# KudanLimited/cuda-bundle-adjustment

Hardware: AMD Instinct MI355X
Metric: ba_edge_iterations_per_sec (higher is better)
Workload: dtype f64

## Files before the change

cuda-bundle-adjustment_amd/csrc/host/c_api.cpp:

```cpp
#include <cmath>
#include <cstring>
#include <deque>
#include <memory>
#include <unordered_map>

#include "../../../include/cugo_hip.h"
#include "../../include/cuda_graph_optimisation.h"
#include "../../include/icp_types.h"
#include "../../include/prior_types.h"
#include "../kernels/kernels.h"
#include "chol_solver.h"
#include "edge_layout.h"
#include "engine.h"
#include "hip_util.h"
#include "rccl_comm.h"
#include "schur_plan.h"

using namespace cugo_host;

namespace
{
template <typename F>
int guarded(F&& f)
{
// ... 311 lines not shown
{
    return guarded([&] { s->analyze(n, rowptr, colind); });
}
int cugo_chol_factor_solve(cugo_chol* s, const double* d_Hsc, double lambda, const double* d_bsc,
                           double* d_x, int32_t* d_fail)
{
    return guarded([&] {
        if (!s->analyzed || !s->ctx)
            throw std::runtime_error("cugo_chol_factor_solve needs an analysed solver with a device context");
        s->factor_solve(d_Hsc, lambda, d_bsc, d_x, d_fail);
    });
}
int cugo_chol_selected_inverse(cugo_chol* s, double* d_sigma)
{
    bool ok = true;
    const int rc = guarded([&] {
        if (!s || !s->ctx || !s->analyzed || !s->factored)
            throw std::runtime_error("cugo_chol_selected_inverse needs a factorisation (cugo_chol_factor_solve) since the "
                                     "last analyze()");
        if (s->own_subtrees())
            throw std::runtime_error("cugo_chol_selected_inverse: not available when the solver factors rank-owned "
                                     "subtrees");
        ok = s->selected_inverse(d_sigma);
    });
    if (rc != CUGO_OK)
        return rc;
    if (!ok)
    {
        set_last_error("cugo_chol_selected_inverse: the factorisation hit a zero pivot");
        return CUGO_ERR_NUMERIC;
    }
    return CUGO_OK;
}
#ifdef CUGO_DEBUG_HOOKS
int cugo_debug_pin_reference(void)
{
    return guarded([&] { cugo_debug_pin_reference_solver(); });
}
int cugo_debug_dump_call(int which, int call, const char* path)
{
    return guarded([&] {
        cugo_chol* s = cugo_debug_solver(which);
        if (!s)
            throw std::runtime_error("cugo_debug_dump_call: no solver has run with CUGO_DEBUG_KEEP");
        s->dump_slot(call, path);
    });
}
int cugo_debug_plan_array(int which, const char* name, const int32_t** out)
{
    cugo_chol* s = cugo_debug_solver(which);
    if (!s)
        return -1;
    return cugo_chol_plan_array(s, name, out);
}
int cugo_debug_dump(const char* dir, int* n_calls)
{
    return guarded([&] {
        const int n = cugo_debug_dump_last_solver(dir);
        if (n_calls)
            *n_calls = n;
    });
}
#endif
int cugo_chol_stats(const cugo_chol* s, double* nnzL, double* flops, int* n_super, int* n_stages,
                    double* front_bytes)
{
// ... 694 lines not shown
```

cuda-bundle-adjustment_amd/csrc/host/chol_solver.cpp:

```cpp
#include "chol_solver.h"

#include <cstdio>
#include <cstdlib>
#include <cstring>
#include <string>

using namespace cugo_host;

void cugo_chol::pack()
{
    const CholPlan& P = plan;
    pack32.clear(), pack64.clear();
    auto put32 = [this](const std::vector<int32_t>& v) {
        const size_t o = pack32.size();
        pack32.insert(pack32.end(), v.begin(), v.end());
        pack32.resize((pack32.size() + 3) & ~size_t(3));
        return o;
    };
    auto put64 = [this](const std::vector<int64_t>& v) {
        const size_t o = pack64.size();
        pack64.insert(pack64.end(), v.begin(), v.end());
        pack64.resize((pack64.size() + 1) & ~size_t(1));
        return o;
    };
    const size_t o_ncb = put32(P.ncb), o_nb = put32(P.nb), o_col0 = put32(P.col0);
    const size_t o_alias = put32(P.alias_of), o_bwnp = put32(P.bw_np), o_lanp = put32(P.la_np);
    const size_t o_rows_ptr = put32(P.rows_ptr), o_rows = put32(P.rows);
    const size_t o_child_ptr = put32(P.child_ptr), o_child = put32(P.child);
    const size_t o_rel_ptr = put32(P.rel_ptr), o_rel = put32(P.rel);
    const size_t o_task_ptr = put32(P.task_ptr), o_task_fronts = put32(P.task_fronts);
    const size_t o_blk_front = put32(P.blk_front), o_blk_row = put32(P.blk_row), o_blk_col = put32(P.blk_col);
    const size_t o_perm = put32(P.perm), o_col_front = put32(P.col_front), o_wl = put32(P.wl);
    const size_t ntask = P.task_ptr.empty() ? 0 : P.task_ptr.size() - 1;
    constexpr int R = cugo_k::EA1_REC;
// ... 85 lines not shown
    }
    for (size_t k = 0; k < P.bc_seg.size() / 3; k++)
        std::memcpy(bc_seg.data() + 4 * k, P.bc_seg.data() + 3 * k, 3 * sizeof(int32_t));
    const size_t o_bc_rec = put32(bc_rec), o_bc_seg = put32(bc_seg);
    const size_t o_asm_map = put32(P.asm_map);
    const size_t o_trans = pack32.size();
    pack32.resize(o_trans + (P.blk_trans.size() + 3) / 4 + 4, 0);
    if (!P.blk_trans.empty())
        std::memcpy(pack32.data() + o_trans, P.blk_trans.data(), P.blk_trans.size());
    const size_t o_asm_off = put64(P.asm_off);
    const size_t o_off = put64(P.off), o_woff = put64(P.woff), o_l21off = put64(P.l21off), o_ldf = put64(P.ldf);
    po = {o_ncb, o_nb, o_col0, o_alias, o_bwnp, o_lanp, o_rows_ptr, o_rows, o_child_ptr, o_child, o_rel_ptr, o_rel,
          o_task_ptr, o_task_fronts, o_blk_front, o_blk_row, o_blk_col, o_perm, o_col_front, o_wl, o_ea1, o_tmeta,
          o_fat, o_asm_map, o_trans, o_asm_off, o_off, o_woff, o_l21off, o_ldf, o_bc_rec, o_bc_seg};
}

void cugo_chol::upload(hipStream_t s)
{
    const CholPlan& P = plan;
    const size_t o_ncb = po[0], o_nb = po[1], o_col0 = po[2], o_alias = po[3], o_bwnp = po[4], o_lanp = po[5];
    const size_t o_rows_ptr = po[6], o_rows = po[7], o_child_ptr = po[8], o_child = po[9], o_rel_ptr = po[10];
    const size_t o_rel = po[11], o_task_ptr = po[12], o_task_fronts = po[13], o_blk_front = po[14], o_blk_row = po[15];
    const size_t o_blk_col = po[16], o_perm = po[17], o_col_front = po[18], o_wl = po[19], o_ea1 = po[20];
    const size_t o_tmeta = po[21], o_fat = po[22], o_asm_map = po[23], o_trans = po[24], o_asm_off = po[25];
    const size_t o_off = po[26], o_woff = po[27], o_l21off = po[28], o_ldf = po[29];
    const size_t o_bc_rec = po[30], o_bc_seg = po[31];
    d_pack32.upload(pack32, s), d_pack64.upload(pack64, s);
    d_fronts.resize((size_t)P.front_doubles + 16);
    d_fronts.zero(s);
    d_xnew.resize((size_t)6 * P.n + 16);
    d_junk.resize(64 * 1024);
    d_winv.resize((size_t)P.winv_doubles + 16);
    d_l21.resize((size_t)P.l21_doubles + 16);
    bw_chain = opt.bw_chain && !opt.lookahead && !P.has_subtree_stage && !P.bc_front.empty();
    if (bw_chain)
    {
        d_bc_state.resize((size_t)cugo_k::BC_DONE + P.n_super);
        d_bc_state.zero(s);
        h_bc_error.resize(1);
        h_bc_error[0] = 0;
        bc_base = 0, bc_epoch = 0;
    }
    CUGO_HIP(hipStreamSynchronize(s));

    cugo_k::CholPlanDev& D = dev;
    D.n_fronts = P.n_super;
    const int32_t* b32 = d_pack32.data();
    const int64_t* b64 = d_pack64.data();
    D.ncb = b32 + o_ncb, D.nb = b32 + o_nb, D.off = b64 + o_off, D.col0 = b32 + o_col0;
    D.rows_ptr = b32 + o_rows_ptr, D.rows = b32 + o_rows;
    D.child_ptr = b32 + o_child_ptr, D.child = b32 + o_child;
    D.rel_ptr = b32 + o_rel_ptr, D.rel = b32 + o_rel;
    D.n_stages = P.n_stages;
    D.task_ptr = b32 + o_task_ptr, D.task_fronts = b32 + o_task_fronts, D.tmeta = b32 + o_tmeta;
    D.n_hsc_blocks = (int)P.blk_front.size();
    D.blk_front = b32 + o_blk_front, D.blk_row = b32 + o_blk_row;
    D.blk_col = b32 + o_blk_col, D.blk_trans = reinterpret_cast<const uint8_t*>(b32 + o_trans);
    D.n = P.n, D.perm = b32 + o_perm, D.col_front = b32 + o_col_front;
    D.junk = d_junk.data();
    D.woff = b64 + o_woff, D.winv = d_winv.data(), D.nc_max = P.nc_max;
    D.ea_lds = opt.ea_lds, D.panel16 = opt.panel16, D.ea_direct = opt.ea_direct;
#ifdef CUGO_DEBUG_HOOKS
    {
        const char* ka = std::getenv("CUGO_KERNEL_ACQUIRE");
        D.kernel_acquire = ka ? std::atoi(ka) & 7 : 0;
        const char* ed = std::getenv("CUGO_DEBUG_DELAY");
        D.dbg_delay = ed ? std::atoi(ed) : 0;
        const char* ez = std::getenv("CUGO_DEBUG_ZERO_LDS");
        D.zero_lds = ez ? std::atoi(ez) : 0, D.lds_doubles = 0;
        D.dbg_skip_wg = -1;
    }
#endif
    D.l21off = b64 + o_l21off, D.l21 = d_l21.data();
    D.ldf = b64 + o_ldf, D.alias_of = b32 + o_alias, D.bw_np = b32 + o_bwnp, D.la_np = b32 + o_lanp;
// ... 136 lines not shown
                    if (plan.woff[k] <= e && plan.woff[k] >= plan.woff[f])
                        f = k;
                stale_line = c.d_winv.data() + e, stale_stage = stage_of[f], stale_kind = 0;
            }
            else if (kind == 1 && e + 16 <= 6LL * plan.n)
                stale_line = c.d_xnew.data() + e, stale_stage = stage_of[plan.col_front[e / 6]], stale_kind = 1;
            if (stale_line)
            {
                c.dbg_scratch.resize(16);
                CUGO_HIP(hipMemcpyAsync(c.dbg_scratch.data(), stale_line, 16 * sizeof(double), hipMemcpyDeviceToDevice, s));
            }
        }
    }
    ~cugo_chol_hooks()
    {
        if (skip_on)
            cugo_k::chol_dbg_skip_end();
    }
    void hash(int slot, const double* ptr, size_t n)
    {
        if (c.dbg_hash && slot < 64)
            cugo_k::launch_hash_words(s, ptr, n, c.dbg_hash + slot);
    }
    void after_level(int st)
    {
        if (hash_levels && st < 24)
        {
            hash(16 + st, c.d_winv.data(), (size_t)c.plan.winv_doubles);
            hash(40 + st, c.d_fronts.data(), (size_t)c.plan.front_doubles);
        }
        if (gap)
            cugo_k::launch_nop(s);
    }
    double* stale_for_potrf(int st) const { return stale_kind == 0 && stale_stage == st ? stale_line : nullptr; }
    void after_two_phase(int st)
    {
        if (stale_kind == 0 && stale_stage == st)
            cugo_k::launch_swap16(s, stale_line, c.dbg_scratch.data());
    }
    void after_backward(int st)
    {
        if (stale_kind == 1 && (st == stale_stage || st == stale_stage - 1))
            cugo_k::launch_swap16(s, stale_line, c.dbg_scratch.data());
    }
    void keep_arrays(double* d_x)
    {
        if (!keep_on || c.dbg_calls > 16)
            return;
        const cugo_host::CholPlan& plan = c.plan;
        const size_t nf = (size_t)plan.front_doubles, nw = (size_t)plan.winv_doubles, nl = (size_t)plan.l21_doubles,
                     nx = (size_t)6 * plan.n;
        while (c.keep.size() < (size_t)c.dbg_calls)
            c.keep.emplace_back(new cugo_host::DevBuf<double>());
        auto& k = *c.keep[c.dbg_calls - 1];
        k.resize(nf + nw + nl + 2 * nx + 8);
        double* dst = k.data();
        const std::pair<const double*, size_t> parts[] = {{c.d_fronts.data(), nf}, {c.d_winv.data(), nw}, {c.d_l21.data(), nl},
                                                          {c.d_xnew.data(), nx}, {d_x, nx}};
        for (const auto& pr : parts)
        {
            if (pr.second)
                CUGO_HIP(hipMemcpyAsync(dst, pr.first, pr.second * sizeof(double), hipMemcpyDeviceToDevice, s));
            dst += pr.second;
        }
        g_last_kept = &c;
    }
};
#define CUGO_HOOK(expr) expr
#else
cugo_chol::~cugo_chol() {}
#define CUGO_HOOK(expr) ((void)0)
#endif

void cugo_chol::factor_solve(const double* d_Hsc, double lambda, const double* d_bsc, double* d_x,
                             int32_t* d_fail)
{
    hipStream_t s = ctx->stream;
    check_chain_error();
    factored = true, last_fail = d_fail;
#ifdef CUGO_DEBUG_HOOKS
    cugo_chol_hooks hooks(*this);
#endif
#ifdef CUGO_STAMPS
    static const bool dbg = std::getenv("CUGO_DEBUG_STAMPS") != nullptr;
    static long long* d_stamps = nullptr;
    if (dbg && !d_stamps)
    {
        CUGO_HIP(hipMalloc(reinterpret_cast<void**>(&d_stamps), 64 * sizeof(long long)));
        CUGO_HIP(hipMemset(d_stamps, 0, 64 * sizeof(long long)));
        cugo_k::set_debug_stamps(d_stamps);
    }
#endif
    cugo_k::launch_chol_assemble(s, dev, d_fronts.data(), (size_t)plan.front_doubles, d_Hsc, lambda, d_bsc, d_fail,
                                 d_wl_ptr + 3L * plan.clr0, plan.nclr, asm_fronts ? d_wl_ptr + 3L * plan.asm0 : nullptr,
                                 plan.nasm);
    CUGO_HOOK(hooks.hash(11, d_fronts.data(), (size_t)plan.front_doubles));
    int pend0 = 0, npend = 0, pend_tile = 64;
    for (int st = 0; st < plan.n_stages; st++)
    {
        const int t0 = plan.stage_task_ptr[st], t1 = plan.stage_task_ptr[st + 1];
        if (plan.has_subtree_stage && st == 0)
            cugo_k::launch_chol_subtree_stage(s, dev, d_fronts.data(), t0, t1 - t0, lds_factor, d_fail);
        else if (lookahead)
        {
            cugo_k::launch_chol_potrf_la(s, dev, d_fronts.data(), t0, t1 - t0, d_wl_ptr + 3L * pend0, npend,
                                         pend_tile, d_fail);
            cugo_k::launch_chol_lead(s, dev, d_fronts.data(), d_wl_ptr + 3L * plan.lead_ptr[st],
                                     plan.lead_ptr[st + 1] - plan.lead_ptr[st], d_wl_ptr + 3L * plan.ea_ptr[st],
                                     plan.ea_ptr[st + 1] - plan.ea_ptr[st], d_wl_ptr + 3L * plan.eab_ptr[st],
                                     plan.eab_ptr[st + 1] - plan.eab_ptr[st]);
            pend0 = plan.sb_ptr[st], npend = plan.sb_ptr[st + 1] - plan.sb_ptr[st];
            pend_tile = plan.stage_tile[st] ? plan.stage_tile[st] : 64;
        }
        else
        {
            double* stale = nullptr;
            double* stale_scratch = nullptr;
            CUGO_HOOK((stale = hooks.stale_for_potrf(st), stale_scratch = dbg_scratch.data()));
            cugo_k::launch_chol_upper_stage(
                s, dev, d_fronts.data(), t0, t1 - t0, d_wl_ptr, plan.ea_ptr[st],
                plan.ea_ptr[st + 1] - plan.ea_ptr[st], plan.eab_ptr[st],
                plan.eab_ptr[st + 1] - plan.eab_ptr[st], plan.syrk_ptr[st],
                plan.syrk_ptr[st + 1] - plan.syrk_ptr[st], plan.stage_tile[st], lds_factor, d_fail, stale, stale_scratch);
            if (plan.stage_tile[st] == 0)
            {
                cugo_k::launch_chol_two_phase(s, dev, d_fronts.data(), d_wl_ptr + 3L * plan.trsm_ptr[st],
                                              plan.trsm_ptr[st + 1] - plan.trsm_ptr[st],
                                              d_wl_ptr + 3L * plan.syrk_ptr[st],
                                              plan.syrk_ptr[st + 1] - plan.syrk_ptr[st]);
                CUGO_HOOK(hooks.after_two_phase(st));
            }
        }
        CUGO_HOOK(hooks.after_level(st));
        bool grouped = false;
        for (size_t k = 0; k < plan.xu_front.size(); k++)
            if (plan.xu_stage[k] == st)
            {
                if (!grouped && bcast_group)
                    bcast_group(true), grouped = true;
                const int f = plan.xu_front[k];
                const int64_t ld = plan.ldf[f], c0 = 6LL * plan.ncb[f], c1 = 6LL * plan.nb[f];
                if (c1 > c0)
                    bcast(d_fronts.data() + plan.off[f] + c0 * ld + c0, (size_t)((c1 - 1 - c0) * ld + c1 + 1 - c0),
                          plan.xu_owner[k]);
            }
        if (grouped)
            bcast_group(false);
    }
    if (npend > 0)
        cugo_k::launch_chol_potrf_la(s, dev, d_fronts.data(), 0, 0, d_wl_ptr + 3L * pend0, npend, pend_tile, d_fail);
    CUGO_HOOK(hooks.hash(12, d_winv.data(), (size_t)plan.winv_doubles));
    CUGO_HOOK(hooks.hash(13, d_l21.data(), (size_t)plan.l21_doubles));
    CUGO_HOOK(hooks.hash(14, d_fronts.data(), (size_t)plan.front_doubles));
    if (bw_chain)
    {
        const int nf = (int)plan.bc_front.size();
        if (++bc_epoch == 0)
            bc_epoch = 1;
        cugo_k::launch_chol_backward_chain(s, dev, d_fronts.data(), nf, d_xnew.data(), d_x, d_bc_state.data(), bc_base,
                                           bc_epoch, d_fail, h_bc_error.data());
        bc_base += (uint32_t)nf;
#ifdef CUGO_STAMPS
        if (dbg)
        {
            static int chain_calls = 0;
            static long long* d_cs = nullptr;
            if (++chain_calls == 4)
            {
                CUGO_HIP(hipMalloc(reinterpret_cast<void**>(&d_cs), 3 * sizeof(long long) * (size_t)nf));
                CUGO_HIP(hipMemset(d_cs, 0, 3 * sizeof(long long) * (size_t)nf));
                cugo_k::set_chain_stamps(d_cs);
            }
            if (chain_calls == 5)
            {
                std::vector<long long> h(3 * (size_t)nf);
                std::vector<int> ticket(plan.n_super, -1);
                for (int t = 0; t < nf; t++)
                    ticket[plan.bc_front[t]] = t;
                CUGO_HIP(hipStreamSynchronize(s));
                CUGO_HIP(hipMemcpy(h.data(), d_cs, h.size() * sizeof(long long), hipMemcpyDeviceToHost));
                cugo_k::set_chain_stamps(nullptr);
                long long first = h[0], last = 0;
                for (int t = 0; t < nf; t++)
                    first = std::min(first, h[3 * t]), last = std::max(last, h[3 * t + 2]);
                std::printf("chain stamps: %d fronts, first start to last done %lld ticks (10 ns)\n", nf, last - first);
                for (int f = plan.bc_front[nf - 1]; f >= 0; f = plan.sparent[f])
                {
                    const int t = ticket[f], pa = plan.sparent[f];
                    std::printf("  front %d ticket %d ncb %d rows %d: start +%lld", f, t, plan.ncb[f], plan.nb[f] - plan.ncb[f],
                                h[3 * t] - first);
                    if (pa >= 0)
                        std::printf(" wait %lld work %lld", h[3 * t + 1] - h[3 * ticket[pa] + 2], h[3 * t + 2] - h[3 * t + 1]);
                    std::printf(" done +%lld\n", h[3 * t + 2] - first);
// ... 121 lines not shown
```

cuda-bundle-adjustment_amd/csrc/host/chol_solver.h:

```cpp
#pragma once
#include "../kernels/kernels.h"
#include "chol_symbolic.h"
#include "hip_util.h"
#include "options.h"

#include <array>
#include <functional>
#include <memory>

struct cugo_chol
{
    cugo_ctx* ctx = nullptr;
    bool analyzed = false;
    cugo_host::Options opt = cugo_host::Options::from_env();
    cugo_host::CholPlan plan;
    std::vector<int32_t> trans32;
    std::vector<int32_t> asm_info;
    std::vector<int32_t> ea1;
    cugo_k::CholPlanDev dev{};
    size_t lds_factor = 0, lds_backward = 0;
    bool lookahead = false;
    bool asm_fronts = true;

    std::vector<int32_t> pack32;
    std::vector<int64_t> pack64;
    std::array<size_t, 32> po{};
    cugo_host::DevBuf<int32_t> d_pack32;
    cugo_host::DevBuf<int64_t> d_pack64;
    const int32_t* d_wl_ptr = nullptr;
    cugo_host::DevBuf<double> d_fronts, d_xnew, d_junk, d_winv, d_l21;
    bool bw_chain = false;
    cugo_host::DevBuf<uint32_t> d_bc_state;
    cugo_host::PinnedBuf<uint32_t> h_bc_error;
    uint32_t bc_base = 0, bc_epoch = 0;
    void check_chain_error();

    int rank = 0, world = 1;
    std::function<void(double*, size_t, int)> bcast;
    std::function<void(bool)> bcast_group;
    ~cugo_chol();
#ifdef CUGO_DEBUG_HOOKS
    unsigned long long* dbg_hash = nullptr;
    int dbg_calls = 0;
    std::vector<std::unique_ptr<cugo_host::DevBuf<double>>> keep;
    cugo_host::DevBuf<double> dbg_scratch;
    void dump_kept(const char* dir);
    void dump_slot(int call, const char* path);
#endif
    bool own_subtrees() const { return bcast && plan.owned; }

    const int32_t* last_fail = nullptr;
    bool factored = false;
    bool si_ready = false;
    cugo_host::DevBuf<double> d_sig;
    cugo_host::DevBuf<int64_t> d_sinfo;
    cugo_host::DevBuf<int32_t> d_sitems;
    std::vector<int32_t> si_ptr;
    bool selected_inverse(double* d_sigma);

    void analyze(int n, const int32_t* rowptr, const int32_t* colind);
    void analyze_host(int n, const int32_t* rowptr, const int32_t* colind);
    void pack();
    void upload(hipStream_t s);
    void factor_solve(const double* d_Hsc, double lambda, const double* d_bsc, double* d_x,
                      int32_t* d_fail);
};

#ifdef CUGO_DEBUG_HOOKS
// ... 5 lines not shown
```

cuda-bundle-adjustment_amd/csrc/host/options.h:

```cpp
#pragma once
#include <cstdlib>

namespace cugo_host
{

struct Options
{
    int hsc_mfma = 1;
    bool hsc_xcd = true;
    bool hsc_rows = false, hsc_strip = false, schur_plan = false;
    bool fuse_t = true;
    bool pose_schur = true;
    bool float32 = false;
    bool speculate = true, trial_event = true, trial_poll = true;
    bool trial_from_build = true;
    bool profile = false;
    bool init_timing = false;
    bool structure_reuse = true;
    bool flatten_reuse = true;
    bool async_structure = true;
    bool host_structure = false;
    bool upload_thread = true;
    int own_subtrees = -1;
    double own_min_gflop = 3.0;
    bool lookahead = false;
    bool ea_lds = true, panel16 = true, asm_fronts = true;
    bool ea_direct = true;
    bool bw_chain = true;
    bool reduce_scatter = true;

    static Options from_env()
    {
        Options o;
        auto flag = [](const char* name) { return std::getenv(name) != nullptr; };
        auto off = [](const char* name) {
            const char* e = std::getenv(name);
            return e && e[0] == '0';
        };
        auto on = [](const char* name) {
            const char* e = std::getenv(name);
            return e && e[0] == '1';
        };
        if (const char* e = std::getenv("CUGO_HSC_MFMA"))
            o.hsc_mfma = e[0] == '0' ? 0 : e[0] == '2' ? 2 : 1;
        o.hsc_xcd = !off("CUGO_HSC_XCD");
        o.schur_plan = flag("CUGO_SCHUR_PLAN");
        o.hsc_rows = on("CUGO_HSC_ROWS"), o.hsc_strip = on("CUGO_HSC_STRIP");
        o.fuse_t = !off("CUGO_FUSE_T");
        o.pose_schur = !off("CUGO_POSE_SCHUR");
        o.float32 = on("CUGO_FLOAT32");
        o.speculate = !off("CUGO_SPECULATE"), o.trial_event = !off("CUGO_TRIAL_EVENT"), o.trial_poll = !off("CUGO_TRIAL_POLL");
        o.trial_from_build = !off("CUGO_TRIAL_FROM_BUILD");
        o.profile = flag("CUGO_PROFILE");
        o.init_timing = flag("CUGO_INIT_TIMING");
        o.structure_reuse = !flag("CUGO_NO_STRUCTURE_REUSE");
        o.flatten_reuse = !flag("CUGO_NO_FLATTEN_REUSE");
        o.async_structure = !off("CUGO_ASYNC_STRUCTURE");
        o.host_structure = flag("CUGO_HOST_STRUCTURE");
        o.upload_thread = !off("CUGO_UPLOAD_THREAD");
        if (const char* e = std::getenv("CUGO_OWN_SUBTREES"))
            o.own_subtrees = e[0] == '1' ? 1 : e[0] == '0' ? 0 : -1;
        if (const char* e = std::getenv("CUGO_OWN_MIN_GFLOP"))
            o.own_min_gflop = std::atof(e);
        if (const char* e = std::getenv("CUGO_LOOKAHEAD"))
            o.lookahead = std::atoi(e) != 0;
        o.ea_lds = !off("CUGO_EA_LDS"), o.panel16 = !off("CUGO_PANEL16"), o.asm_fronts = !off("CUGO_ASM_FRONTS");
        o.ea_direct = !off("CUGO_EA_DIRECT");
        o.bw_chain = !off("CUGO_BW_CHAIN");
        o.reduce_scatter = !off("CUGO_REDUCE_SCATTER");
        return o;
    }
};

}
```

cuda-bundle-adjustment_amd/csrc/kernels/chol_kernels.hip:

```cpp
#include <algorithm>
#include <cstdio>

#include "kernels.h"

namespace
{

constexpr int CBS = 256;
constexpr double PIVOT_TOL = 1e-14;
constexpr int TR = 64;
constexpr int NC_MAX = 96;
constexpr int LLD = NC_MAX + 17;
constexpr int PW = 6;

using cugo_k::CholPlanDev;
typedef double double4_t __attribute__((ext_vector_type(4)));

__device__ __forceinline__ void assemble_scatter(const CholPlanDev& p, double* __restrict__ fronts,
                                                 const double* __restrict__ Hsc, double lambda,
                                                 const double* __restrict__ bsc, int32_t* __restrict__ fail, int nblk,
                                                 int bid)
{
    if (bid >= nblk)
    {
// ... 26 lines not shown
        if (r == c)
            v += lambda;
        F[(6L * cb + c) * ld + 6L * rb + r] = v;
    }
    else if (!p.blk_trans[k])
        F[(6L * cb + c) * ld + 6L * rb + r] = v;
    else
        F[(6L * cb + r) * ld + 6L * rb + c] = v;
}

__global__ __launch_bounds__(CBS) void k_assemble_blocks(CholPlanDev p, double* __restrict__ fronts,
                                                         const double* __restrict__ Hsc,
                                                         double lambda, const double* __restrict__ bsc,
                                                         int32_t* __restrict__ fail, int nblk)
{
    assemble_scatter(p, fronts, Hsc, lambda, bsc, fail, nblk, (int)blockIdx.x);
}

__global__ __launch_bounds__(CBS) void k_clear_fronts(CholPlanDev p, double* __restrict__ fronts,
                                                      const int32_t* __restrict__ items)
{
    const int32_t* it = items + 3 * blockIdx.x;
    const int f = it[0], c0 = it[1], c1 = it[2];
    const long ld = p.ldf[f];
    const int nrows = 6 * p.nb[f] + 1;
    double* F = fronts + p.off[f];
    for (int r = c0 + threadIdx.x; r < nrows; r += CBS)
#pragma unroll 4
        for (int c = c0; c < c1; c++)
            if (r >= c)
                F[(long)c * ld + r] = 0.0;
}

__global__ __launch_bounds__(CBS) void k_assemble_fronts(CholPlanDev p, double* __restrict__ fronts,
                                                         const double* __restrict__ Hsc, double lambda,
                                                         const double* __restrict__ bsc, int32_t* __restrict__ fail,
                                                         int item0, int nzero, int nblk)
{
    if ((int)blockIdx.x >= nzero)
    {
        assemble_scatter(p, fronts, Hsc, lambda, bsc, fail, nblk, (int)blockIdx.x - nzero);
        return;
    }
    const int32_t* it = p.fat + 16L * (item0 + (int)blockIdx.x);
    const int4 h0 = *reinterpret_cast<const int4*>(it), h1 = *reinterpret_cast<const int4*>(it + 4);
    const long off = *reinterpret_cast<const int64_t*>(it + 8), ld = *reinterpret_cast<const int64_t*>(it + 10);
    const int cb0 = h0.y, cb1 = h0.z, nb = h1.y;
    const int nrows = 6 * nb + 1;
    double* F = fronts + off;
    if (!h1.x)
    {
        for (int r = 6 * cb0 + threadIdx.x; r < nrows; r += CBS)
            for (int c = 6 * cb0; c < 6 * cb1; c++)
                if (r >= c)
                    F[(long)c * ld + r] = 0.0;
        return;
    }
    const int32_t* map = p.asm_map + (long)(uint32_t)h1.z + ((long)h1.w << 32);
    for (int r = 6 * cb0 + threadIdx.x; r < nrows; r += CBS)
    {
        const int rb = r / 6, i = r - 6 * rb;
        for (int cb = cb0; cb < cb1; cb++)
        {
            if (rb < cb)
                continue;
            const int taken = rb == nb ? map[cb] : map[nb + cb * nb - cb * (cb - 1) / 2 + (rb - cb)];
            if (taken >= 0)
                continue;
            double* Fc = F + 6L * cb * ld + r;
#pragma unroll
            for (int c = 0; c < 6; c++)
                if (rb > cb || i >= c)
                    Fc[c * ld] = 0.0;
        }
    }
}

#ifdef CUGO_STAMPS
__device__ long long* g_stamps = nullptr;
__device__ int g_stamp_block[8] = {0, 0, 0, 0, 1, 0, 0, 0};
__device__ __forceinline__ void stamp(int kernel, int slot)
{
    if (g_stamps && (int)blockIdx.x == g_stamp_block[kernel] && threadIdx.x == 0)
        g_stamps[kernel * 8 + slot] = clock64();
}
__device__ __forceinline__ void stamp_value(int kernel, int slot, long long v)
{
    if (g_stamps && (int)blockIdx.x == g_stamp_block[kernel] && threadIdx.x == 0)
        g_stamps[kernel * 8 + slot] = v;
}
#else
__device__ __forceinline__ void stamp(int, int) {}
__device__ __forceinline__ void stamp_value(int, int, long long) {}
#endif


__device__ __forceinline__ void wave_lds_sync()
{
    __builtin_amdgcn_fence(__ATOMIC_ACQ_REL, "workgroup");
    __builtin_amdgcn_wave_barrier();
}

__device__ __forceinline__ void ea_chunk(const double* __restrict__ U, long ldc, int nru, int nbr,
                                         const int32_t* __restrict__ rel, double* __restrict__ Fp,
                                         long ldp, long rhs_row, int jb, int ch, int lane,
                                         double* __restrict__ sink, double* dsink, int rbeg, int rend)
{
    const int i = rbeg + 64 * ch + lane;
// ... 2061 lines not shown
        g_bc_stamps[3 * ticket + slot] = (long long)__builtin_amdgcn_s_memrealtime();
}
#else
__device__ __forceinline__ void bc_stamp(int, int) {}
#endif
constexpr unsigned long long BW_SPIN_TICKS = 25000000ULL;

__device__ __forceinline__ void bw_wait(gu32* word, unsigned epoch, gu32* st, int32_t* fail, unsigned* h_error)
{
    if (__hip_atomic_load(word, __ATOMIC_RELAXED, __HIP_MEMORY_SCOPE_AGENT) == epoch)
        return;
    const unsigned long long t0 = __builtin_amdgcn_s_memrealtime();
    for (;;)
    {
        __builtin_amdgcn_s_sleep(1);
        if (__hip_atomic_load(word, __ATOMIC_RELAXED, __HIP_MEMORY_SCOPE_AGENT) == epoch)
            return;
        if (__hip_atomic_load(st + cugo_k::BC_ABORT, __ATOMIC_RELAXED, __HIP_MEMORY_SCOPE_AGENT) != 0)
            return;
        if (__builtin_amdgcn_s_memrealtime() - t0 > BW_SPIN_TICKS)
        {
            __hip_atomic_store(st + cugo_k::BC_ABORT, 1u, __ATOMIC_RELAXED, __HIP_MEMORY_SCOPE_AGENT);
            __hip_atomic_store(st + cugo_k::BC_ERROR, 1u, __ATOMIC_RELAXED, __HIP_MEMORY_SCOPE_AGENT);
            __hip_atomic_store(fail, 1, __ATOMIC_RELAXED, __HIP_MEMORY_SCOPE_AGENT);
            __hip_atomic_store(h_error, 1u, __ATOMIC_RELAXED, __HIP_MEMORY_SCOPE_SYSTEM);
            return;
        }
    }
}

__global__ __launch_bounds__(BIG) void k_backward_chain(CholPlanDev p, const double* __restrict__ fronts,
                                                        double* xnew, double* __restrict__ xout, unsigned* state,
                                                        unsigned ticket_base, unsigned epoch, int32_t* fail,
                                                        unsigned* h_error)
{
    kernel_acquire(p);
    extern __shared__ double lds[];
    dbg_fill_lds(p, lds);
    gu32* st = (gu32*)state;
    double* vs = lds;
    int* tk = reinterpret_cast<int*>(lds + NC_MAX);
    if (threadIdx.x == 0)
        *tk = (int)(__hip_atomic_fetch_add(st + cugo_k::BC_HEAD, 1u, __ATOMIC_RELAXED, __HIP_MEMORY_SCOPE_AGENT) - ticket_base);
    __syncthreads();
    const int t = __builtin_amdgcn_readfirstlane(*tk);
    if (t < 0 || t >= (int)gridDim.x)
        return;
#ifdef CUGO_DEBUG_HOOKS
    const bool skip = p.dbg_skip_wg == t;
#else
    const bool skip = false;
#endif
    bc_stamp(t, 0);
    const int32_t* rc = p.bc_rec + cugo_k::BC_REC * t;
    const int f = rc[0], ncb = rc[1], nb = rc[2], c0 = rc[3], nseg = rc[6];
    const int32_t* rows = p.rows + rc[4];
    const int32_t* sg = p.bc_seg + 4 * rc[5];
    const long* r64 = reinterpret_cast<const long*>(rc + 8);
    const long l21o = r64[1], ld = r64[3];
    const int ncs = 6 * ncb, nrs = 6 * (nb - ncb), ncp = pad16(ncs);
    const double* L = l21o >= 0 ? p.l21 + l21o : fronts + r64[2] + ncs;
    const long ldl = l21o >= 0 ? nrs + 1 : ld;
    const double* Wg = p.winv + r64[0];
    const int g = threadIdx.x >> 3, l8 = threadIdx.x & 7;
    const bool colok = g < ncs;
    const int j = min(g, ncs - 1);
    const double* col = L + (long)j * ldl;
    const double* wcol = Wg + (long)j * ncp;
    const int jb = j / 6, comp = j - 6 * jb;
    double wv[12];
    const int k0 = (j & ~15) + 2 * l8;
#pragma unroll
    for (int u = 0; u < 6; u++)
    {
        const double2 v = *reinterpret_cast<const double2*>(wcol + min(k0 + 16 * u, ncp - 2));
        wv[2 * u] = v.x, wv[2 * u + 1] = v.y;
    }
    const double y = col[nrs];
    const int pj = p.perm[c0 + jb];
// ... 172 lines not shown
}
size_t chol_lds_potrf_bytes()
{
    return std::max((size_t)NC_MAX * LLD + NC_MAX + (NC_MAX >> 4) * (16 * 17) + 8, (size_t)p16::LDS_DOUBLES + 8) *
           sizeof(double);
}
int chol_max_pivot_cols() { return NC_MAX; }
size_t chol_lds_backward_bytes(int nc_max, long ld_max)
{
    const size_t ncp = (size_t)((nc_max + 15) & ~15);
    return (ncp + (size_t)ld_max + 8) * sizeof(double);
}

void set_debug_stamps(long long* d_buf)
{
#ifdef CUGO_STAMPS
    (void)hipMemcpyToSymbol(HIP_SYMBOL(g_stamps), &d_buf, sizeof(d_buf));
#else
    (void)d_buf;
#endif
}
void set_chain_stamps(long long* d_buf)
{
#ifdef CUGO_STAMPS
    (void)hipMemcpyToSymbol(HIP_SYMBOL(g_bc_stamps), &d_buf, sizeof(d_buf));
#else
    (void)d_buf;
#endif
}

void launch_chol_assemble(hipStream_t s, const CholPlanDev& p, double* d_fronts,
                          size_t front_doubles, const double* d_Hsc, double lambda,
                          const double* d_bsc, int32_t* d_fail, const int32_t* d_clear_items, int nclear,
                          const int32_t* d_asm_items, int nasm)
{
    if (d_asm_items && nasm > 0)
    {
        const long n = 36L * p.n_hsc_blocks;
        const int nblk = (int)((n + CBS - 1) / CBS), nrhs = std::max(1, (6 * p.n + CBS - 1) / CBS);
        CUGO_LAUNCH(k_assemble_fronts, dim3(nasm + nblk + nrhs), dim3(CBS), 0, s, p, d_fronts, d_Hsc, lambda, d_bsc,
                    d_fail, (int)((d_asm_items - p.wl_base) / 3), nasm, nblk);
        return;
    }
    if (nclear > 0)
        CUGO_LAUNCH(k_clear_fronts, dim3(nclear), dim3(CBS), 0, s, p, d_fronts, d_clear_items);
    else
        (void)hipMemsetAsync(d_fronts, 0, front_doubles * sizeof(double), s);
    const long n = 36L * p.n_hsc_blocks;
    const int nblk = (int)((n + CBS - 1) / CBS), nrhs = std::max(1, (6 * p.n + CBS - 1) / CBS);
    CUGO_LAUNCH(k_assemble_blocks, dim3(nblk + nrhs), dim3(CBS), 0, s, p, d_fronts, d_Hsc, lambda, d_bsc, d_fail,
                nblk);
}

void launch_chol_subtree_stage(hipStream_t s, const CholPlanDev& p, double* d_fronts, int task0,
                               int ntasks, size_t lds_bytes, int32_t* d_fail)
{
    if (ntasks <= 0)
        return;
    ensure_lds(reinterpret_cast<const void*>(k_subtree_factor), lds_bytes);
    CUGO_LAUNCH(k_subtree_factor, dim3(ntasks), dim3(BIG), lds_bytes, s, p, d_fronts, task0,
                       d_fail);
}

void launch_chol_two_phase(hipStream_t s, const CholPlanDev& p, double* d_fronts, const int32_t* d_trsm, int ntrsm,
                           const int32_t* d_syrk, int nsyrk)
{
    const size_t lds_t = (size_t)NC_MAX * PSTB * sizeof(double), lds_s = (size_t)2 * KC_SYRK2 * PST * sizeof(double);
    if (ntrsm > 0)
    {
        ensure_lds(reinterpret_cast<const void*>(k_up_trsm), lds_t);
        CUGO_LAUNCH(k_up_trsm, dim3(ntrsm), dim3(BIG), lds_t, s, with_lds(p, lds_t, "k_up_trsm", ntrsm), d_fronts, d_trsm);
    }
    if (nsyrk > 0)
    {
// ... 93 lines not shown
{
    const long total = 36L * B + 6L * n;
    if (total > 0)
        CUGO_LAUNCH(k_xs_pack, dim3((unsigned)((total + CBS - 1) / CBS)), dim3(CBS), 0, s, d_off, B, n, d_sys, d_xbuf);
}
void launch_xs_unpack(hipStream_t s, const int64_t* d_off, int B, int n, const double* d_xbuf, double* d_sys, long lo,
                      long hi, long top0)
{
    const long total = 36L * B + 6L * n;
    if (total > 0)
        CUGO_LAUNCH(k_xs_unpack, dim3((unsigned)((total + CBS - 1) / CBS)), dim3(CBS), 0, s, d_off, B, n, d_xbuf, d_sys,
                    lo, hi, top0);
}

void launch_chol_unpermute(hipStream_t s, const CholPlanDev& p, const double* d_xnew, double* d_x)
{
    if (p.n > 0)
        CUGO_LAUNCH(k_unpermute, dim3((6 * p.n + CBS - 1) / CBS), dim3(CBS), 0, s, p, d_xnew, d_x);
}

void launch_chol_backward_stage(hipStream_t s, const CholPlanDev& p, double* d_fronts, int task0,
                                int ntasks, size_t lds_bytes, double* d_xnew, double* d_x,
                                const int32_t* d_wl_gemv, int ngemv)
{
    if (ntasks <= 0)
        return;
    ensure_lds(reinterpret_cast<const void*>(k_backward_stage), lds_bytes);
    CUGO_LAUNCH(k_backward_stage, dim3(ntasks + ngemv), dim3(BIG), lds_bytes, s, with_lds(p, lds_bytes, "k_backward_stage", ntasks + ngemv, ntasks), d_fronts, task0,
                       ntasks, d_wl_gemv, d_xnew, d_x);
}

void launch_chol_backward_chain(hipStream_t s, const CholPlanDev& p, double* d_fronts, int nfronts, double* d_xnew,
                                double* d_x, uint32_t* d_state, uint32_t ticket_base, uint32_t epoch, int32_t* d_fail,
                                uint32_t* h_error)
{
    if (nfronts <= 0)
        return;
    const size_t lds_bytes = 96 * 1024;
    ensure_lds(reinterpret_cast<const void*>(k_backward_chain), lds_bytes);
    CUGO_LAUNCH(k_backward_chain, dim3(nfronts), dim3(BIG), lds_bytes, s, with_lds(p, lds_bytes, "k_backward_chain", nfronts),
                d_fronts, d_xnew, d_x, d_state, ticket_base, epoch, d_fail, h_error);
}

}
```

cuda-bundle-adjustment_amd/csrc/kernels/kernels.h:

```cpp
#pragma once
#include <hip/hip_runtime.h>
#include <stddef.h>
#include <stdint.h>

#include "../../../include/cugo_hip.h"

namespace cugo_k
{

struct LaunchHook
{
    virtual void begin(const char* kernel, hipStream_t s) = 0;
    virtual void end(const char* kernel, hipStream_t s) = 0;
    virtual ~LaunchHook() {}
};
void set_launch_hook(LaunchHook* h);
LaunchHook* launch_hook();
struct LaunchScope
{
    const char* name;
    hipStream_t s;
    LaunchHook* h;
    LaunchScope(const char* n, hipStream_t st) : name(n), s(st), h(launch_hook())
    {
// ... 130 lines not shown
#endif
    const int32_t* col0;
    const int32_t* rows_ptr;
    const int32_t* rows;
    const int32_t* child_ptr;
    const int32_t* child;
    const int32_t* rel_ptr;
    const int32_t* rel;
    int n_stages;
    const int32_t* ea1;
    const int32_t* tmeta;
    const int32_t* asm_map;
    const int64_t* asm_off;
    const int32_t* wl_base;
    const int32_t* fat;
    const int32_t* bc_rec;
    const int32_t* bc_seg;
    const int32_t* task_ptr;
    const int32_t* task_fronts;
    int n_hsc_blocks;
    const int32_t* blk_front;
    const int32_t* blk_row;
    const int32_t* blk_col;
    const uint8_t* blk_trans;
    int n;
    const int32_t* perm;
    const int32_t* col_front;
    double* junk;
};

void launch_chol_assemble(hipStream_t s, const CholPlanDev& p, double* d_fronts, size_t front_doubles,
                          const double* d_Hsc, double lambda, const double* d_bsc, int32_t* d_fail,
                          const int32_t* d_clear_items, int nclear, const int32_t* d_asm_items = nullptr,
                          int nasm = 0);
void launch_chol_subtree_stage(hipStream_t s, const CholPlanDev& p, double* d_fronts, int task0,
                               int ntasks, size_t lds_bytes, int32_t* d_fail);
void launch_chol_upper_stage(hipStream_t s, const CholPlanDev& p, double* d_fronts, int task0,
                             int ntasks, const int32_t* d_wl, int eap0, int neap, int ea0, int nea,
                             int sy0, int nsy, int tile, size_t lds_bytes, int32_t* d_fail,
                             double* dbg_line = nullptr, double* dbg_scratch = nullptr);
#ifdef CUGO_DEBUG_HOOKS
void launch_swap16(hipStream_t s, double* line, double* scratch);
#endif
void launch_chol_two_phase(hipStream_t s, const CholPlanDev& p, double* d_fronts, const int32_t* d_trsm, int ntrsm,
                           const int32_t* d_syrk, int nsyrk);
void launch_chol_potrf_la(hipStream_t s, const CholPlanDev& p, double* d_fronts, int task0, int ntasks,
                          const int32_t* d_tiles, int ntiles, int tile, int32_t* d_fail);
void launch_chol_lead(hipStream_t s, const CholPlanDev& p, double* d_fronts, const int32_t* d_lead,
                      int nlead, const int32_t* d_eap, int neap, const int32_t* d_eab, int neab);
void launch_chol_backward_stage(hipStream_t s, const CholPlanDev& p, double* d_fronts, int task0,
                                int ntasks, size_t lds_bytes, double* d_xnew, double* d_x,
                                const int32_t* d_wl_gemv, int ngemv);
constexpr int BC_REC = 16, BC_HEAD = 0, BC_ABORT = 32, BC_ERROR = 33, BC_DONE = 64;
void launch_chol_backward_chain(hipStream_t s, const CholPlanDev& p, double* d_fronts, int nfronts, double* d_xnew,
                                double* d_x, uint32_t* d_state, uint32_t ticket_base, uint32_t epoch, int32_t* d_fail,
                                uint32_t* h_error);
#ifdef CUGO_DEBUG_HOOKS
void launch_nop(hipStream_t s);
void chol_dbg_skip_begin(int target_launch, int target_wg, const char* dump_path);
void chol_dbg_skip_end();
void launch_hash_words(hipStream_t s, const void* p, size_t n_words, unsigned long long* out);
#endif
void launch_flag_to_double(hipStream_t s, int32_t* d_flag);
void launch_chol_unpermute(hipStream_t s, const CholPlanDev& p, const double* d_xnew, double* d_x);
void launch_xs_pack(hipStream_t s, const int64_t* d_off, int B, int n, const double* d_sys, double* d_xbuf);
void launch_xs_unpack(hipStream_t s, const int64_t* d_off, int B, int n, const double* d_xbuf, double* d_sys, long lo,
                      long hi, long top0);
void set_debug_stamps(long long* d_buf);
void set_chain_stamps(long long* d_buf);
size_t chol_lds_factor_bytes(int nc_max);
size_t chol_lds_backward_bytes(int nc_max, long ld_max);
int chol_max_pivot_cols();

void launch_selinv_rows(hipStream_t s, const CholPlanDev& p, const double* d_fronts, double* d_sig,
                        const int64_t* d_sinfo, const int32_t* d_items, int nitems);
void launch_selinv_jj(hipStream_t s, const CholPlanDev& p, const double* d_fronts, double* d_sig, int task0,
                      int ntasks);
void launch_selinv_subtree(hipStream_t s, const CholPlanDev& p, const double* d_fronts, double* d_sig,
                           const int64_t* d_sinfo, int task0, int ntasks);
void launch_selinv_gather(hipStream_t s, const CholPlanDev& p, const double* d_sig, double* d_out);
int selinv_row_tile();
void launch_cov_pose_diag(hipStream_t s, int P, const int32_t* d_rowptr, const double* d_sigma, double* d_out);
void launch_lm_covariance(hipStream_t s, int L, const int32_t* d_lm_ptr, const int32_t* d_e_pose,
                          const uint8_t* d_flags, const double* d_Hll, const double* d_Hpl, const int32_t* d_rowptr,
                          const int32_t* d_colind, const double* d_sigma, double* d_out, int32_t* d_fail);

}
```

include/cugo_hip.h:

```cpp
#ifndef CUGO_HIP_H
#define CUGO_HIP_H

#include <stddef.h>
#include <stdint.h>

#ifdef __cplusplus
extern "C" {
#endif

#define CUGO_OK 0
#define CUGO_ERR_NO_DEVICE (-1)
#define CUGO_ERR_HIP (-2)
#define CUGO_ERR_INVALID (-3)
#define CUGO_ERR_NUMERIC (-4)

enum { CUGO_RK_NONE = 0, CUGO_RK_CAUCHY = 1, CUGO_RK_TUKEY = 2,
       CUGO_RK_HUBER = 3  };

enum
{
    CUGO_EDGE_FIXED_L = 1,
    CUGO_EDGE_FIXED_P = 2,
    CUGO_EDGE_STEREO = 4,
    CUGO_EDGE_INACTIVE = 8
// ... 65 lines not shown
    int n_groups;
    int n_slots, n_rhs;
    const int32_t* d_grp_ptr;
    const int32_t* d_grp_nwave;
    const int32_t* d_slot_rhs;
    const int32_t* d_slot_ptr;
    const uint16_t* d_prod;
    const int32_t* d_red_ptr;
    const int32_t* d_red_slot;
    const int32_t* d_blk_pose;
    double* d_part_H;
    double* d_part_b;
} cugo_hsc_struct;

typedef struct cugo_hsc_plan cugo_hsc_plan;
int cugo_hsc_plan_create(cugo_ctx* ctx, int n_edges, int n_poses_free, const int32_t* h_pose,
                         const int32_t* h_lm, const uint8_t* h_flags, const int32_t* h_rowptr,
                         const int32_t* h_colind, cugo_hsc_struct* hs, cugo_hsc_plan** out);
void cugo_hsc_plan_destroy(cugo_hsc_plan* plan);

int cugo_compute_schur(cugo_ctx* ctx, const cugo_edges* ev, const cugo_hsc_struct* hs,
                       double lambda, int damp_hsc_diag, const double* d_Hpp, const double* d_bp,
                       const double* d_Hll, const double* d_bl, const void* d_Hpl,
                       double* d_invHll, void* d_T, double* d_bsc, double* d_Hsc);

typedef struct cugo_chol cugo_chol;
int cugo_chol_create(cugo_ctx* ctx, cugo_chol** out);
void cugo_chol_destroy(cugo_chol* s);
int cugo_chol_analyze(cugo_chol* s, int n_block_rows, const int32_t* h_rowptr,
                      const int32_t* h_colind);
int cugo_chol_factor_solve(cugo_chol* s, const double* d_Hsc, double lambda, const double* d_bsc,
                           double* d_x, int32_t* d_fail);
int cugo_chol_selected_inverse(cugo_chol* s, double* d_sigma);
int cugo_chol_stats(const cugo_chol* s, double* nnzL, double* flops, int* n_supernodes,
                    int* n_stages, double* front_bytes);
int cugo_chol_plan_sizes(const cugo_chol* s, int* n, int* n_super, int* n_rows_total);
int cugo_chol_plan_get(const cugo_chol* s, int32_t* perm, int32_t* super_ptr, int32_t* rows_ptr,
                       int32_t* rows, int32_t* parent);
int cugo_chol_plan_array(cugo_chol* s, const char* name, const int32_t** out);
int cugo_chol_plan_array64(cugo_chol* s, const char* name, const int64_t** out);

int cugo_backsubst_update(cugo_ctx* ctx, const cugo_edges* ev, double lambda,
                          const double* d_invHll, const double* d_bl, const double* d_bp,
                          const void* d_Hpl, const double* d_xp, double* d_xl,
                          const double* d_poses_in, const double* d_lms_in, double* d_poses_out,
                          double* d_lms_out, double* d_scale);

typedef struct cugo_icp_edges
{
    int n_poses_total, n_poses_free;
    int n_plane;
    const int32_t* d_plane_pose;
    const int32_t* d_plane_pose_ptr;
    const double* d_plane_p;
    const double* d_plane_nd;
    const double* d_plane_omega;
    int n_plane_omega;
    const uint8_t* d_plane_flags;
    int rk_plane;
    double delta_plane;
    int n_line;
    const int32_t* d_line_pose;
    const int32_t* d_line_pose_ptr;
    const double* d_line_p;
    const double* d_line_au;
    const double* d_line_omega;
// ... 119 lines not shown
```

Before: 640.0 million.

## Prefill next call's front zeroing with spare workgroups in backward chain

Adds extra 'rider' workgroups to the backward-substitution chain kernel. They use compute units left idle by the chain to zero and prefill the assembly fronts for the next factorisation. The next assemble launch then skips its zeroing blocks. This relies on the fronts not being read after the backward pass, and the feature is gated to configurations where that holds. It also adds API functions for copying factors back and zeroes the W/L21 buffers at upload.

```diff
diff --git a/cuda-bundle-adjustment_amd/csrc/host/c_api.cpp b/cuda-bundle-adjustment_amd/csrc/host/c_api.cpp
--- a/cuda-bundle-adjustment_amd/csrc/host/c_api.cpp
+++ b/cuda-bundle-adjustment_amd/csrc/host/c_api.cpp
@@ -367,6 +367,24 @@
     }
     return CUGO_OK;
 }
+int64_t cugo_chol_factor_copy(cugo_chol* s, int which, double* h_out, int64_t capacity)
+{
+    int64_t n = -1;
+    const int rc = guarded([&] {
+        if (!s || !s->ctx || !s->analyzed)
+            throw std::runtime_error("cugo_chol_factor_copy needs an analysed solver with a device context");
+        const cugo_host::DevBuf<double>* src = which == 0 ? &s->d_winv : which == 1 ? &s->d_l21 : which == 2 ? &s->d_fronts : nullptr;
+        const int64_t len = which == 0 ? s->plan.winv_doubles : which == 1 ? s->plan.l21_doubles : s->plan.front_doubles;
+        if (!src)
+            throw std::runtime_error("cugo_chol_factor_copy: which must be 0 (W), 1 (L21) or 2 (fronts)");
+        CUGO_HIP(hipStreamSynchronize(s->ctx->stream));
+        if (h_out && capacity >= len && len > 0)
+            CUGO_HIP(hipMemcpy(h_out, src->data(), (size_t)len * sizeof(double), hipMemcpyDeviceToHost));
+        n = len;
+    });
+    return rc == CUGO_OK ? n : -1;
+}
+int cugo_chol_fronts_prefilled(const cugo_chol* s) { return s && s->fronts_prefilled ? 1 : 0; }
 #ifdef CUGO_DEBUG_HOOKS
 int cugo_debug_pin_reference(void)
 {
diff --git a/cuda-bundle-adjustment_amd/csrc/host/chol_solver.cpp b/cuda-bundle-adjustment_amd/csrc/host/chol_solver.cpp
--- a/cuda-bundle-adjustment_amd/csrc/host/chol_solver.cpp
+++ b/cuda-bundle-adjustment_amd/csrc/host/chol_solver.cpp
@@ -1,5 +1,6 @@
 #include "chol_solver.h"
 
+#include <algorithm>
 #include <cstdio>
 #include <cstdlib>
 #include <cstring>
@@ -151,6 +152,7 @@
     d_junk.resize(64 * 1024);
     d_winv.resize((size_t)P.winv_doubles + 16);
     d_l21.resize((size_t)P.l21_doubles + 16);
+    d_winv.zero(s), d_l21.zero(s);
     bw_chain = opt.bw_chain && !opt.lookahead && !P.has_subtree_stage && !P.bc_front.empty();
     if (bw_chain)
     {
@@ -159,6 +161,16 @@
         h_bc_error.resize(1);
         h_bc_error[0] = 0;
         bc_base = 0, bc_epoch = 0;
+    }
+    fronts_prefilled = false, fill_riders = 0;
+    if (opt.bw_fill && bw_chain && opt.asm_fronts && P.nasm > 0 && !P.owned && P.xu_front.empty() && P.xx_lo.empty() &&
+        std::all_of(P.bc_front.begin(), P.bc_front.end(), [&](int f) { return P.l21off[f] >= 0; }))
+    {
+        int ncu = 0;
+        CUGO_HIP(hipDeviceGetAttribute(&ncu, hipDeviceAttributeMultiprocessorCount, ctx ? ctx->device : 0));
+        const int spare = ncu - (int)P.bc_front.size();
+        if (spare >= ncu / 4)
+            fill_riders = spare;
     }
     CUGO_HIP(hipStreamSynchronize(s));
 
@@ -361,6 +373,7 @@
         if (gap)
             cugo_k::launch_nop(s);
     }
+    bool keeps_fronts() const { return keep_on || skip_on || stale_line != nullptr; }
     double* stale_for_potrf(int st) const { return stale_kind == 0 && stale_stage == st ? stale_line : nullptr; }
     void after_two_phase(int st)
     {
@@ -422,7 +435,8 @@
 #endif
     cugo_k::launch_chol_assemble(s, dev, d_fronts.data(), (size_t)plan.front_doubles, d_Hsc, lambda, d_bsc, d_fail,
                                  d_wl_ptr + 3L * plan.clr0, plan.nclr, asm_fronts ? d_wl_ptr + 3L * plan.asm0 : nullptr,
-                                 plan.nasm);
+                                 plan.nasm, fronts_prefilled);
+    fronts_prefilled = false;
     CUGO_HOOK(hooks.hash(11, d_fronts.data(), (size_t)plan.front_doubles));
     int pend0 = 0, npend = 0, pend_tile = 64;
     for (int st = 0; st < plan.n_stages; st++)
@@ -486,8 +500,12 @@
         const int nf = (int)plan.bc_front.size();
         if (++bc_epoch == 0)
             bc_epoch = 1;
+        int riders = fill_riders;
+        CUGO_HOOK(riders = hooks.keeps_fronts() ? 0 : riders);
         cugo_k::launch_chol_backward_chain(s, dev, d_fronts.data(), nf, d_xnew.data(), d_x, d_bc_state.data(), bc_base,
-                                           bc_epoch, d_fail, h_bc_error.data());
+                                           bc_epoch, d_fail, h_bc_error.data(), d_wl_ptr + 3L * plan.asm0, plan.nasm,
+                                           riders);
+        fronts_prefilled = riders > 0;
         bc_base += (uint32_t)nf;
 #ifdef CUGO_STAMPS
         if (dbg)
diff --git a/cuda-bundle-adjustment_amd/csrc/host/chol_solver.h b/cuda-bundle-adjustment_amd/csrc/host/chol_solver.h
--- a/cuda-bundle-adjustment_amd/csrc/host/chol_solver.h
+++ b/cuda-bundle-adjustment_amd/csrc/host/chol_solver.h
@@ -34,6 +34,8 @@
     cugo_host::PinnedBuf<uint32_t> h_bc_error;
     uint32_t bc_base = 0, bc_epoch = 0;
     void check_chain_error();
+    int fill_riders = 0;
+    bool fronts_prefilled = false;
 
     int rank = 0, world = 1;
     std::function<void(double*, size_t, int)> bcast;
diff --git a/cuda-bundle-adjustment_amd/csrc/host/options.h b/cuda-bundle-adjustment_amd/csrc/host/options.h
--- a/cuda-bundle-adjustment_amd/csrc/host/options.h
+++ b/cuda-bundle-adjustment_amd/csrc/host/options.h
@@ -27,6 +27,7 @@
     bool ea_lds = true, panel16 = true, asm_fronts = true;
     bool ea_direct = true;
     bool bw_chain = true;
+    bool bw_fill = true;
     bool reduce_scatter = true;
 
     static Options from_env()
@@ -67,6 +68,7 @@
         o.ea_lds = !off("CUGO_EA_LDS"), o.panel16 = !off("CUGO_PANEL16"), o.asm_fronts = !off("CUGO_ASM_FRONTS");
         o.ea_direct = !off("CUGO_EA_DIRECT");
         o.bw_chain = !off("CUGO_BW_CHAIN");
+        o.bw_fill = !off("CUGO_BW_FILL");
         o.reduce_scatter = !off("CUGO_REDUCE_SCATTER");
         return o;
     }
diff --git a/cuda-bundle-adjustment_amd/csrc/kernels/chol_kernels.hip b/cuda-bundle-adjustment_amd/csrc/kernels/chol_kernels.hip
--- a/cuda-bundle-adjustment_amd/csrc/kernels/chol_kernels.hip
+++ b/cuda-bundle-adjustment_amd/csrc/kernels/chol_kernels.hip
@@ -82,17 +82,9 @@
                 F[(long)c * ld + r] = 0.0;
 }
 
-__global__ __launch_bounds__(CBS) void k_assemble_fronts(CholPlanDev p, double* __restrict__ fronts,
-                                                         const double* __restrict__ Hsc, double lambda,
-                                                         const double* __restrict__ bsc, int32_t* __restrict__ fail,
-                                                         int item0, int nzero, int nblk)
-{
-    if ((int)blockIdx.x >= nzero)
-    {
-        assemble_scatter(p, fronts, Hsc, lambda, bsc, fail, nblk, (int)blockIdx.x - nzero);
-        return;
-    }
-    const int32_t* it = p.fat + 16L * (item0 + (int)blockIdx.x);
+__device__ __forceinline__ void assemble_zero_item(const CholPlanDev& p, double* __restrict__ fronts, int item, int tid)
+{
+    const int32_t* it = p.fat + 16L * item;
     const int4 h0 = *reinterpret_cast<const int4*>(it), h1 = *reinterpret_cast<const int4*>(it + 4);
     const long off = *reinterpret_cast<const int64_t*>(it + 8), ld = *reinterpret_cast<const int64_t*>(it + 10);
     const int cb0 = h0.y, cb1 = h0.z, nb = h1.y;
@@ -100,14 +92,14 @@
     double* F = fronts + off;
     if (!h1.x)
     {
-        for (int r = 6 * cb0 + threadIdx.x; r < nrows; r += CBS)
+        for (int r = 6 * cb0 + tid; r < nrows; r += CBS)
             for (int c = 6 * cb0; c < 6 * cb1; c++)
                 if (r >= c)
                     F[(long)c * ld + r] = 0.0;
         return;
     }
     const int32_t* map = p.asm_map + (long)(uint32_t)h1.z + ((long)h1.w << 32);
-    for (int r = 6 * cb0 + threadIdx.x; r < nrows; r += CBS)
+    for (int r = 6 * cb0 + tid; r < nrows; r += CBS)
     {
         const int rb = r / 6, i = r - 6 * rb;
         for (int cb = cb0; cb < cb1; cb++)
@@ -124,6 +116,19 @@
                     Fc[c * ld] = 0.0;
         }
     }
+}
+
+__global__ __launch_bounds__(CBS) void k_assemble_fronts(CholPlanDev p, double* __restrict__ fronts,
+                                                         const double* __restrict__ Hsc, double lambda,
+                                                         const double* __restrict__ bsc, int32_t* __restrict__ fail,
+                                                         int item0, int nzero, int nblk)
+{
+    if ((int)blockIdx.x >= nzero)
+    {
+        assemble_scatter(p, fronts, Hsc, lambda, bsc, fail, nblk, (int)blockIdx.x - nzero);
+        return;
+    }
+    assemble_zero_item(p, fronts, item0 + (int)blockIdx.x, (int)threadIdx.x);
 }
 
 #ifdef CUGO_STAMPS
@@ -2251,9 +2256,18 @@
 __global__ __launch_bounds__(BIG) void k_backward_chain(CholPlanDev p, const double* __restrict__ fronts,
                                                         double* xnew, double* __restrict__ xout, unsigned* state,
                                                         unsigned ticket_base, unsigned epoch, int32_t* fail,
-                                                        unsigned* h_error)
+                                                        unsigned* h_error, int nf, int fill_item0, int fill_items)
 {
     kernel_acquire(p);
+    if ((int)blockIdx.x >= nf)
+    {
+        const int sub = (int)threadIdx.x / CBS, nsub = BIG / CBS;
+        const int stride = ((int)gridDim.x - nf) * nsub;
+        for (int it = ((int)blockIdx.x - nf) * nsub + sub; it < fill_items; it += stride)
+            assemble_zero_item(p, const_cast<double*>(fronts), fill_item0 + it, (int)threadIdx.x % CBS);
+        kernel_release(p);
+        return;
+    }
     extern __shared__ double lds[];
     dbg_fill_lds(p, lds);
     gu32* st = (gu32*)state;
@@ -2263,7 +2277,7 @@
         *tk = (int)(__hip_atomic_fetch_add(st + cugo_k::BC_HEAD, 1u, __ATOMIC_RELAXED, __HIP_MEMORY_SCOPE_AGENT) - ticket_base);
     __syncthreads();
     const int t = __builtin_amdgcn_readfirstlane(*tk);
-    if (t < 0 || t >= (int)gridDim.x)
+    if (t < 0 || t >= nf)
         return;
 #ifdef CUGO_DEBUG_HOOKS
     const bool skip = p.dbg_skip_wg == t;
@@ -2502,14 +2516,15 @@
 void launch_chol_assemble(hipStream_t s, const CholPlanDev& p, double* d_fronts,
                           size_t front_doubles, const double* d_Hsc, double lambda,
                           const double* d_bsc, int32_t* d_fail, const int32_t* d_clear_items, int nclear,
-                          const int32_t* d_asm_items, int nasm)
+                          const int32_t* d_asm_items, int nasm, bool zeros_done)
 {
     if (d_asm_items && nasm > 0)
     {
         const long n = 36L * p.n_hsc_blocks;
         const int nblk = (int)((n + CBS - 1) / CBS), nrhs = std::max(1, (6 * p.n + CBS - 1) / CBS);
-        CUGO_LAUNCH(k_assemble_fronts, dim3(nasm + nblk + nrhs), dim3(CBS), 0, s, p, d_fronts, d_Hsc, lambda, d_bsc,
-                    d_fail, (int)((d_asm_items - p.wl_base) / 3), nasm, nblk);
+        const int nzero = zeros_done ? 0 : nasm;
+        CUGO_LAUNCH(k_assemble_fronts, dim3(nzero + nblk + nrhs), dim3(CBS), 0, s, p, d_fronts, d_Hsc, lambda, d_bsc,
+                    d_fail, (int)((d_asm_items - p.wl_base) / 3), nzero, nblk);
         return;
     }
     if (nclear > 0)
@@ -2669,14 +2684,18 @@
 
 void launch_chol_backward_chain(hipStream_t s, const CholPlanDev& p, double* d_fronts, int nfronts, double* d_xnew,
                                 double* d_x, uint32_t* d_state, uint32_t ticket_base, uint32_t epoch, int32_t* d_fail,
-                                uint32_t* h_error)
+                                uint32_t* h_error, const int32_t* d_fill_items, int nfill_items, int nriders)
 {
     if (nfronts <= 0)
         return;
+    if (!d_fill_items || nfill_items <= 0)
+        nriders = 0;
     const size_t lds_bytes = 96 * 1024;
     ensure_lds(reinterpret_cast<const void*>(k_backward_chain), lds_bytes);
-    CUGO_LAUNCH(k_backward_chain, dim3(nfronts), dim3(BIG), lds_bytes, s, with_lds(p, lds_bytes, "k_backward_chain", nfronts),
-                d_fronts, d_xnew, d_x, d_state, ticket_base, epoch, d_fail, h_error);
-}
-
-}
+    CUGO_LAUNCH(k_backward_chain, dim3(nfronts + nriders), dim3(BIG), lds_bytes, s,
+                with_lds(p, lds_bytes, "k_backward_chain", nfronts + nriders), d_fronts, d_xnew, d_x, d_state, ticket_base,
+                epoch, d_fail, h_error, nfronts, nriders ? (int)((d_fill_items - p.wl_base) / 3) : 0,
+                nriders ? nfill_items : 0);
+}
+
+}
diff --git a/cuda-bundle-adjustment_amd/csrc/kernels/kernels.h b/cuda-bundle-adjustment_amd/csrc/kernels/kernels.h
--- a/cuda-bundle-adjustment_amd/csrc/kernels/kernels.h
+++ b/cuda-bundle-adjustment_amd/csrc/kernels/kernels.h
@@ -186,7 +186,7 @@
 void launch_chol_assemble(hipStream_t s, const CholPlanDev& p, double* d_fronts, size_t front_doubles,
                           const double* d_Hsc, double lambda, const double* d_bsc, int32_t* d_fail,
                           const int32_t* d_clear_items, int nclear, const int32_t* d_asm_items = nullptr,
-                          int nasm = 0);
+                          int nasm = 0, bool zeros_done = false);
 void launch_chol_subtree_stage(hipStream_t s, const CholPlanDev& p, double* d_fronts, int task0,
                                int ntasks, size_t lds_bytes, int32_t* d_fail);
 void launch_chol_upper_stage(hipStream_t s, const CholPlanDev& p, double* d_fronts, int task0,
@@ -208,7 +208,8 @@
 constexpr int BC_REC = 16, BC_HEAD = 0, BC_ABORT = 32, BC_ERROR = 33, BC_DONE = 64;
 void launch_chol_backward_chain(hipStream_t s, const CholPlanDev& p, double* d_fronts, int nfronts, double* d_xnew,
                                 double* d_x, uint32_t* d_state, uint32_t ticket_base, uint32_t epoch, int32_t* d_fail,
-                                uint32_t* h_error);
+                                uint32_t* h_error, const int32_t* d_fill_items = nullptr, int nfill_items = 0,
+                                int nriders = 0);
 #ifdef CUGO_DEBUG_HOOKS
 void launch_nop(hipStream_t s);
 void chol_dbg_skip_begin(int target_launch, int target_wg, const char* dump_path);
diff --git a/include/cugo_hip.h b/include/cugo_hip.h
--- a/include/cugo_hip.h
+++ b/include/cugo_hip.h
@@ -121,6 +121,8 @@
 int cugo_chol_factor_solve(cugo_chol* s, const double* d_Hsc, double lambda, const double* d_bsc,
                            double* d_x, int32_t* d_fail);
 int cugo_chol_selected_inverse(cugo_chol* s, double* d_sigma);
+int64_t cugo_chol_factor_copy(cugo_chol* s, int which, double* h_out, int64_t capacity);
+int cugo_chol_fronts_prefilled(const cugo_chol* s);
 int cugo_chol_stats(const cugo_chol* s, double* nnzL, double* flops, int* n_supernodes,
                     int* n_stages, double* front_bytes);
 int cugo_chol_plan_sizes(const cugo_chol* s, int* n, int* n_super, int* n_rows_total);
```

Result: no change. 644.9 million (median of 6 runs) (+0.8%).
